# PaddlePaddle/MetaGym

Measured on NVIDIA H100. Metric: env-steps/sec (quadrotor 6-DoF, 65k envs), higher is better.
Workload: dtype f32

## Files before the change

### include/mgb200.h

```cpp
#ifndef MGB200_H
#define MGB200_H

#include <stdint.h>

#ifdef __cplusplus
extern "C" {
#endif

#define MGB_OK 0
#define MGB_ERR_ARG (-1)
#define MGB_ERR_CUDA (-2)
#define MGB_ERR_STATE (-3)


#define MGB_TASK_NO_COLLISION 0
#define MGB_TASK_HOVERING_CONTROL 1
#define MGB_TASK_VELOCITY_CONTROL 2

#define MGB_INTEGRATOR_REFERENCE 0
#define MGB_INTEGRATOR_RK4 1

#define MGB_FAIL_NONE 0
#define MGB_FAIL_RANGE 1
#define MGB_FAIL_VELOCITY 2
// ... 11 lines not shown
    double fail_velocity, fail_range, fail_w;
    float propeller[12];
    float propeller_norm[4];
    double min_voltage, max_voltage;
    float init_velocity[3];
    double init_velocity_noise;
    float init_angular_velocity[3];
    double init_angular_velocity_noise;
    double dt;
    int32_t nt;
    int32_t task;
    double healthy_reward;
    double z_offset;
    int32_t integrator;
    int32_t rk4_steps;
} mgb_quad_cfg;

typedef struct mgb_quad mgb_quad;

int mgb_quad_create(mgb_quad **out, int64_t n_envs, const mgb_quad_cfg *cfg, int device, int64_t env_index_base);
void mgb_quad_destroy(mgb_quad *h);

int mgb_quad_obs_dim(const mgb_quad *h);
int64_t mgb_quad_num_envs(const mgb_quad *h);

int mgb_quad_set_options(mgb_quad *h, int auto_reset, uint64_t seed);

int mgb_quad_set_map(mgb_quad *h, const int32_t *map_host, int32_t rows, int32_t cols);

int mgb_quad_set_targets(mgb_quad *h, const float *tbl_dev, int32_t n_tasks, const int32_t *env2task_dev);

int mgb_quad_make_targets(mgb_quad *h, const float *act_dev, int32_t n_tasks, float *tbl_dev, void *stream);

int mgb_quad_reset(mgb_quad *h, const uint8_t *mask_dev, const double *noise_dev, float *obs_dev, void *stream);

int mgb_quad_step(mgb_quad *h, const float *act_dev, float *obs_dev, float *rew_dev, uint8_t *done_dev,
                  int32_t *fail_dev, float *final_obs_dev, void *stream);
int mgb_quad_step_ex(mgb_quad *h, const float *act_dev, float *obs_dev, float *rew_dev, uint8_t *done_dev,
                     int32_t *fail_dev, float *final_obs_dev, uint8_t *truncated_dev, void *stream);

int mgb_quad_rollout(mgb_quad *h, int32_t T, const float *act_dev, uint64_t act_seed, float *act_out_dev,
                     float *obs_dev, float *rew_dev, uint8_t *done_dev, void *stream);
int mgb_quad_rollout_ex(mgb_quad *h, int32_t T, const float *act_dev, uint64_t act_seed, float *act_out_dev,
                        float *obs_dev, float *rew_dev, uint8_t *done_dev, float *final_obs_dev, uint8_t *truncated_dev,
                        void *stream);

#define MGB_ACT_TANH 0
#define MGB_ACT_RELU 1
#define MGB_POLICY_SAMPLE 0
#define MGB_POLICY_MEAN 1
#define MGB_POLICY_MAX_HIDDEN 3
#define MGB_POLICY_MAX_WIDTH 64

typedef struct mgb_policy {
    const float *params_dev;
    int32_t n_hidden;
    int32_t width[3];
    int32_t activation;
    int32_t mode;
} mgb_policy;

int mgb_quad_rollout_policy(mgb_quad *h, int32_t T, const mgb_policy *pol, uint64_t seed, float *act_out_dev,
                            float *logp_out_dev, float *obs0_out_dev, float *obs_dev, float *rew_dev, uint8_t *done_dev,
                            float *final_obs_dev, uint8_t *truncated_dev, void *stream);

int mgb_quad_step_host(mgb_quad *h, const float *act_host, float *obs_host, float *rew_host, uint8_t *done_host,
                       int32_t *fail_host, float *final_obs_host, void *stream);
int mgb_quad_step_host_ex(mgb_quad *h, const float *act_host, float *obs_host, float *rew_host, uint8_t *done_host,
                          int32_t *fail_host, float *final_obs_host, uint8_t *truncated_host, void *stream);

int mgb_quad_state(mgb_quad *h, float *state_dev, int32_t *ct_dev, int load, void *stream);

#define MGB_FINGERPRINT_WORDS 4
int64_t mgb_quad_record_bytes(const mgb_quad *h);
int mgb_quad_snapshot(mgb_quad *h, uint8_t *rec_dev, void *stream);
int mgb_quad_restore(mgb_quad *h, const uint8_t *rec_dev, int64_t n_rec, const int64_t *row_of_env_dev, void *stream);
int mgb_quad_counters(mgb_quad *h, uint64_t *t_base, int set);
int mgb_quad_fingerprint(const mgb_quad *h, uint64_t *out);

int64_t mgb_quad_launch_count(const mgb_quad *h);

const char *mgb_quad_step_kernel(const mgb_quad *h);


#define MGB_MAZE_2D 0
#define MGB_MAZE_DISCRETE_3D 1
#define MGB_MAZE_CONTINUOUS_3D 2

#define MGB_MAZE_SURVIVAL 0
#define MGB_MAZE_ESCAPE 1

#define MGB_OBS_U8 0
#define MGB_OBS_I32 1
#define MGB_OBS_F32 2

typedef struct mgb_maze_task_scalars {
    int32_t start[2];
    int32_t goal[2];
    double cell_size, wall_height, agent_height;
    double initial_life, max_life, step_reward, goal_reward;
} mgb_maze_task_scalars;

typedef struct mgb_maze_cfg {
    int32_t kind;
    int32_t task_type;
    int32_t n_cells;
    int32_t max_steps;
    int32_t view_grid;
    int32_t res_h;
    int32_t res_v;
    int32_t obs_dtype;
    double max_vision;
    double fov;
    double l_focal;
    double text_size;
} mgb_maze_cfg;

typedef struct mgb_maze mgb_maze;

int mgb_maze_create(mgb_maze **out, int64_t n_envs, const mgb_maze_cfg *cfg, int device, int64_t env_index_base);
void mgb_maze_destroy(mgb_maze *h);
int64_t mgb_maze_obs_bytes_per_env(const mgb_maze *h);

int mgb_maze_set_textures(mgb_maze *h, const uint8_t *grounds_host, int32_t n_tex, const uint8_t *ceil_host,
                          int32_t tex_size);

int mgb_maze_set_task(mgb_maze *h, int32_t n_tasks, const int8_t *walls_host, const int8_t *texts_host,
                      const double *food_rewards_host, const int32_t *food_interval_host,
                      const mgb_maze_task_scalars *scalars_host, const int32_t *env2task_host);

typedef struct mgb_maze_sampler_cfg {
    int32_t allow_loops, n_texts, food_interval, pad;
    double cell_size, wall_height, agent_height, step_reward;
    double goal_reward;
    double food_reward, initial_life, max_life, food_density, crowd_ratio;
} mgb_maze_sampler_cfg;

int mgb_maze_resample_tasks(mgb_maze *h, const uint8_t *mask_dev, const mgb_maze_sampler_cfg *cfg, uint64_t seed,
                            void *stream);

int mgb_maze_get_tasks(mgb_maze *h, int32_t count, const int32_t *task_slots_host, int8_t *walls_host, int8_t *texts_host,
                       double *food_rewards_host, int32_t *food_interval_host, mgb_maze_task_scalars *scalars_host);

int mgb_maze_set_cache(mgb_maze *h, int enabled);

int mgb_maze_cache_info(const mgb_maze *h, int64_t out[16]);

int mgb_maze_update_tasks(mgb_maze *h, int32_t count, const int32_t *task_slots_host, const int8_t *walls_host,
                          const int8_t *texts_host, const double *food_rewards_host, const int32_t *food_interval_host,
                          const mgb_maze_task_scalars *scalars_host, void *stream);

int mgb_maze_reset(mgb_maze *h, const uint8_t *mask_dev, void *obs_dev, void *stream);

int mgb_maze_step(mgb_maze *h, const void *act_dev, void *obs_dev, double *rew_dev, uint8_t *done_dev,
                  void *final_obs_dev, uint8_t *truncated_dev, void *stream);
int mgb_maze_set_options(mgb_maze *h, int auto_reset);

int mgb_maze_rollout(mgb_maze *h, int32_t T, const void *act_dev, uint64_t act_seed, void *act_out_dev,
                     void *obs_dev, double *rew_dev, uint8_t *done_dev, void *final_obs_dev, uint8_t *truncated_dev,
                     const mgb_maze_sampler_cfg *resample_cfg, uint64_t resample_seed, void *stream);

int mgb_maze_rollout_policy(mgb_maze *h, int32_t T, const mgb_policy *pol, uint64_t seed,
                            const mgb_maze_sampler_cfg *resample_cfg, uint64_t resample_seed, int32_t *act_out_dev,
                            float *logp_out_dev, float *obs0_out_dev, float *obs_dev, double *rew_dev, uint8_t *done_dev,
                            float *final_obs_dev, uint8_t *truncated_dev, void *stream);

// ... 67 lines not shown
```

### metagym_b200/_lib.py

```python
import ctypes
import os

PKG = os.path.dirname(os.path.abspath(__file__))
LIB_PATH = os.path.join(PKG, "libmgb200.so")

c_i32, c_i64, c_u64, c_f32, c_f64 = ctypes.c_int32, ctypes.c_int64, ctypes.c_uint64, ctypes.c_float, ctypes.c_double
vp = ctypes.c_void_p


class MgbError(RuntimeError):
    pass


class QuadCfg(ctypes.Structure):
    _fields_ = [
        ("precision", c_f64), ("quality", c_f64), ("inv_inertia", c_f32 * 9), ("drag_m", c_f32 * 3),
        ("drag_f", c_f32 * 3), ("gravity_center", c_f32 * 3), ("ct", c_f64 * 3), ("mm", c_f64), ("jm", c_f64),
        ("phi", c_f64), ("ra", c_f64), ("fail_velocity", c_f64), ("fail_range", c_f64), ("fail_w", c_f64),
        ("propeller", c_f32 * 12), ("propeller_norm", c_f32 * 4), ("min_voltage", c_f64), ("max_voltage", c_f64),
        ("init_velocity", c_f32 * 3), ("init_velocity_noise", c_f64), ("init_angular_velocity", c_f32 * 3),
        ("init_angular_velocity_noise", c_f64), ("dt", c_f64), ("nt", c_i32), ("task", c_i32),
        ("healthy_reward", c_f64), ("z_offset", c_f64), ("integrator", c_i32), ("rk4_steps", c_i32),
    ]


class MazeTaskScalars(ctypes.Structure):
    _fields_ = [("start", c_i32 * 2), ("goal", c_i32 * 2), ("cell_size", c_f64), ("wall_height", c_f64),
                ("agent_height", c_f64), ("initial_life", c_f64), ("max_life", c_f64), ("step_reward", c_f64),
                ("goal_reward", c_f64)]


class MazeSamplerCfg(ctypes.Structure):
    _fields_ = [("allow_loops", c_i32), ("n_texts", c_i32), ("food_interval", c_i32), ("pad", c_i32),
                ("cell_size", c_f64), ("wall_height", c_f64), ("agent_height", c_f64), ("step_reward", c_f64),
                ("goal_reward", c_f64), ("food_reward", c_f64), ("initial_life", c_f64), ("max_life", c_f64),
                ("food_density", c_f64), ("crowd_ratio", c_f64)]


class MazeCfg(ctypes.Structure):
    _fields_ = [("kind", c_i32), ("task_type", c_i32), ("n_cells", c_i32), ("max_steps", c_i32),
                ("view_grid", c_i32), ("res_h", c_i32), ("res_v", c_i32), ("obs_dtype", c_i32),
                ("max_vision", c_f64), ("fov", c_f64), ("l_focal", c_f64), ("text_size", c_f64)]


class Policy(ctypes.Structure):
    _fields_ = [("params_dev", vp), ("n_hidden", c_i32), ("width", c_i32 * 3), ("activation", c_i32), ("mode", c_i32)]


class RnnPolicy(ctypes.Structure):
    _fields_ = [("params_dev", vp), ("hidden", c_i32), ("feedback", c_i32), ("reset", c_i32), ("head_hidden", c_i32),
                ("head_width", c_i32), ("activation", c_i32), ("mode", c_i32), ("cell", c_i32)]


ACT_TANH, ACT_RELU = 0, 1
POLICY_SAMPLE, POLICY_MEAN = 0, 1
RNN_RESET_EPISODE, RNN_RESET_TASK = 0, 1
RNN_CELL_GRU, RNN_CELL_LSTM = 0, 1


SIGNATURES = {
    "mgb_quad_create": (ctypes.c_int, [ctypes.POINTER(vp), c_i64, ctypes.POINTER(QuadCfg), ctypes.c_int, c_i64]),
    "mgb_quad_destroy": (None, [vp]),
    "mgb_quad_obs_dim": (ctypes.c_int, [vp]),
    "mgb_quad_num_envs": (c_i64, [vp]),
    "mgb_quad_set_options": (ctypes.c_int, [vp, ctypes.c_int, c_u64]),
    "mgb_quad_set_map": (ctypes.c_int, [vp, vp, c_i32, c_i32]),
    "mgb_quad_set_targets": (ctypes.c_int, [vp, vp, c_i32, vp]),
    "mgb_quad_make_targets": (ctypes.c_int, [vp, vp, c_i32, vp, vp]),
    "mgb_quad_reset": (ctypes.c_int, [vp, vp, vp, vp, vp]),
    "mgb_quad_step": (ctypes.c_int, [vp, vp, vp, vp, vp, vp, vp, vp]),
    "mgb_quad_rollout": (ctypes.c_int, [vp, c_i32, vp, c_u64, vp, vp, vp, vp, vp]),
    "mgb_quad_step_host": (ctypes.c_int, [vp, vp, vp, vp, vp, vp, vp, vp]),
    "mgb_quad_step_ex": (ctypes.c_int, [vp, vp, vp, vp, vp, vp, vp, vp, vp]),
    "mgb_quad_step_host_ex": (ctypes.c_int, [vp, vp, vp, vp, vp, vp, vp, vp, vp]),
    "mgb_quad_rollout_ex": (ctypes.c_int, [vp, c_i32, vp, c_u64, vp, vp, vp, vp, vp, vp, vp]),
    "mgb_quad_rollout_policy": (ctypes.c_int, [vp, c_i32, ctypes.POINTER(Policy), c_u64, vp, vp, vp, vp, vp, vp, vp, vp,
                                               vp]),
    "mgb_quad_state": (ctypes.c_int, [vp, vp, vp, ctypes.c_int, vp]),
    "mgb_quad_launch_count": (c_i64, [vp]),
    "mgb_quad_step_kernel": (ctypes.c_char_p, [vp]),
    "mgb_maze_create": (ctypes.c_int, [ctypes.POINTER(vp), c_i64, ctypes.POINTER(MazeCfg), ctypes.c_int, c_i64]),
    "mgb_maze_destroy": (None, [vp]),
    "mgb_maze_obs_bytes_per_env": (c_i64, [vp]),
    "mgb_maze_set_textures": (ctypes.c_int, [vp, vp, c_i32, vp, c_i32]),
    "mgb_maze_set_task": (ctypes.c_int, [vp, c_i32, vp, vp, vp, vp, ctypes.POINTER(MazeTaskScalars), vp]),
    "mgb_maze_resample_tasks": (ctypes.c_int, [vp, vp, ctypes.POINTER(MazeSamplerCfg), c_u64, vp]),
    "mgb_maze_get_tasks": (ctypes.c_int, [vp, c_i32, vp, vp, vp, vp, vp, ctypes.POINTER(MazeTaskScalars)]),
    "mgb_maze_set_cache": (ctypes.c_int, [vp, ctypes.c_int]),
    "mgb_maze_cache_info": (ctypes.c_int, [vp, vp]),
    "mgb_maze_update_tasks": (ctypes.c_int, [vp, c_i32, vp, vp, vp, vp, vp, ctypes.POINTER(MazeTaskScalars), vp]),
    "mgb_maze_reset": (ctypes.c_int, [vp, vp, vp, vp]),
    "mgb_maze_step": (ctypes.c_int, [vp, vp, vp, vp, vp, vp, vp, vp]),
    "mgb_maze_set_options": (ctypes.c_int, [vp, ctypes.c_int]),
    "mgb_peer_alloc": (ctypes.c_int, [ctypes.c_int, c_u64, ctypes.POINTER(ctypes.c_void_p)]),
    "mgb_peer_free": (ctypes.c_int, [ctypes.c_int, vp]),
    "mgb_peer_export": (ctypes.c_int, [ctypes.c_int, vp, vp]),
    "mgb_peer_open": (ctypes.c_int, [ctypes.c_int, vp, ctypes.POINTER(ctypes.c_void_p)]),
    "mgb_peer_close": (ctypes.c_int, [ctypes.c_int, vp]),
    "mgb_quad_set_mirrors": (ctypes.c_int, [vp, ctypes.c_int, vp]),
    "mgb_maze_set_mirrors": (ctypes.c_int, [vp, ctypes.c_int, vp]),
    "mgb_quad_set_mirror_window": (ctypes.c_int, [vp, vp, c_u64]),
    "mgb_maze_set_mirror_window": (ctypes.c_int, [vp, vp, c_u64]),
    "mgb_quad_set_multicast": (ctypes.c_int, [vp, ctypes.c_int64]),
    "mgb_maze_set_multicast": (ctypes.c_int, [vp, ctypes.c_int64]),
    "mgb_maze_rollout": (ctypes.c_int, [vp, c_i32, vp, c_u64, vp, vp, vp, vp, vp, vp, ctypes.POINTER(MazeSamplerCfg),
                                        c_u64, vp]),
    "mgb_maze_rollout_policy": (ctypes.c_int, [vp, c_i32, ctypes.POINTER(Policy), c_u64, ctypes.POINTER(MazeSamplerCfg),
                                               c_u64, vp, vp, vp, vp, vp, vp, vp, vp, vp]),
    "mgb_maze_rollout_rnn": (ctypes.c_int, [vp, c_i32, ctypes.POINTER(RnnPolicy), c_u64, ctypes.POINTER(MazeSamplerCfg),
                                            c_u64, vp, vp, vp, vp, vp, vp, vp, vp, vp, vp, vp, vp]),
    "mgb_maze_pose": (ctypes.c_int, [vp, vp, vp, vp]),
    "mgb_maze_state": (ctypes.c_int, [vp, vp, vp, vp]),
    "mgb_maze_launch_count": (c_i64, [vp]),
    "mgb_maze_god_view": (ctypes.c_int, [vp, c_i32, vp, c_i32, c_i32, vp, vp]),
    "mgb_maze_set_path": (ctypes.c_int, [vp, ctypes.c_int]),
    "mgb_maze_path": (ctypes.c_int, [vp, c_i32, vp, vp, vp, vp]),
    "mgb_quad_record_bytes": (c_i64, [vp]),
    "mgb_quad_snapshot": (ctypes.c_int, [vp, vp, vp]),
    "mgb_quad_restore": (ctypes.c_int, [vp, vp, c_i64, vp, vp]),
    "mgb_quad_counters": (ctypes.c_int, [vp, ctypes.POINTER(c_u64), ctypes.c_int]),
    "mgb_quad_fingerprint": (ctypes.c_int, [vp, ctypes.POINTER(c_u64)]),
    "mgb_maze_record_bytes": (c_i64, [vp]),
    "mgb_maze_snapshot": (ctypes.c_int, [vp, vp, vp]),
    "mgb_maze_restore": (ctypes.c_int, [vp, vp, c_i64, vp, vp]),
    "mgb_maze_counters": (ctypes.c_int, [vp, ctypes.POINTER(c_u64), ctypes.c_int]),
    "mgb_maze_fingerprint": (ctypes.c_int, [vp, ctypes.POINTER(c_u64)]),
    "mgb_last_error": (ctypes.c_char_p, []),
    "mgb_version": (ctypes.c_char_p, []),
    "mgb_device_count": (ctypes.c_int, []),
}

_lib = None


def load():
    global _lib
    if _lib is not None:
        return _lib
    if not os.path.exists(LIB_PATH):
        raise MgbError("%s not found: build it with `python -m metagym_b200._build` (nvcc, sm_90a). "
                       "metagym_b200 has no CPU fallback." % LIB_PATH)
    lib = ctypes.CDLL(LIB_PATH)
    for name, (res, args) in SIGNATURES.items():
        fn = getattr(lib, name)
        fn.restype = res
        fn.argtypes = args
    _lib = lib
    return lib


def check(rc):
    if rc != 0:
        raise MgbError("libmgb200: %s (code %d)" % (load().mgb_last_error().decode(), rc))


def current_stream(torch, device):
    get = getattr(torch._C, "_cuda_getCurrentRawStream", None)
    if get is not None:
        return get(device.index)
    return torch.cuda.current_stream(device).cuda_stream


def ptr(t):
# ... 6 lines not shown
```

### metagym_b200/csrc/quad.cu

```cuda
#include <math.h>
#include <stdlib.h>
#include <string.h>
#include <memory>
#include <new>
#include <type_traits>
#include <utility>
#include <vector>

#include "mgb_common.cuh"
#include "mgb_policy.cuh"
#include "quad_lanes.cuh"

namespace {

constexpr int kThreads = 64;
constexpr int kMaxObs = 19;

struct QuadConst {
    float h;
    float k1phi;
    float k1;
    float inv_phi;
    float hjm;
    float hk;
    float mm;
    float ct0, ct1, ct2;
    float vmin, vmax;
    float A[4], B[4];
    float px[4], py[4], pz[4];
    float Df[3], Dm[3];
    float cg[3];
    float hI[9];
    float gm;
    float c_hm;
    float c_h2m;
    float fail_r2, fail_v2, fail_w2;
    float dt, healthy, z_off;
    float init_v[3], init_w[3], noise_v, noise_w;
    int nt, task, substeps, obs_dim;
    int rk4_steps;
    float rk4_h;
    float inv_jm, inv_m;
    float Iinv[9];
    int simple;
};

struct QuadArgs {
    float4 *planes;
    int64_t n_pad;
    int64_t n;
    int64_t env_base;
    const float *act;
    float *obs;
    float *rew;
    uint8_t *done;
    int32_t *fail;
    float *final_obs;
    const float4 *targets;
    int n_tasks;
    const int32_t *sat;
    int map_rows, map_cols, x_off, y_off;
    const int32_t *env2task;
    uint64_t seed;
    int auto_reset;
    int per_cta;
    int T;
    uint64_t act_seed;
    uint32_t t_base;
    float *act_out;
    MgbMirrors mir;
    uint8_t *truncated;
};

template <class T> struct VState {
    T p[3], v[3], om[3], w[4], R[9];
    int ct[Lanes<T>::N], ep[Lanes<T>::N];
};
using QState = VState<float>;

constexpr int kTileEnvs = 128;
constexpr int kPlanes = 6;

__device__ __forceinline__ float4 *tile_base(const QuadArgs &a, int64_t e)
{
    return a.planes + (e / kTileEnvs) * (kPlanes * kTileEnvs) + (e % kTileEnvs);
}

__device__ __forceinline__ void unpack_state(const float4 q[kPlanes], QState &s)
{
    s.p[0] = q[0].x; s.p[1] = q[0].y; s.p[2] = q[0].z; s.v[0] = q[0].w;
    s.v[1] = q[1].x; s.v[2] = q[1].y; s.om[0] = q[1].z; s.om[1] = q[1].w;
    s.om[2] = q[2].x; s.w[0] = q[2].y; s.w[1] = q[2].z; s.w[2] = q[2].w;
    s.w[3] = q[3].x; s.R[0] = q[3].y; s.R[1] = q[3].z; s.R[2] = q[3].w;
    s.R[3] = q[4].x; s.R[4] = q[4].y; s.R[5] = q[4].z; s.R[6] = q[4].w;
    s.R[7] = q[5].x; s.R[8] = q[5].y; s.ct[0] = __float_as_int(q[5].z); s.ep[0] = __float_as_int(q[5].w);
}
__device__ __forceinline__ void pack_state(const QState &s, float4 q[kPlanes])
{
    q[0] = make_float4(s.p[0], s.p[1], s.p[2], s.v[0]);
    q[1] = make_float4(s.v[1], s.v[2], s.om[0], s.om[1]);
    q[2] = make_float4(s.om[2], s.w[0], s.w[1], s.w[2]);
    q[3] = make_float4(s.w[3], s.R[0], s.R[1], s.R[2]);
    q[4] = make_float4(s.R[3], s.R[4], s.R[5], s.R[6]);
    q[5] = make_float4(s.R[7], s.R[8], __int_as_float(s.ct[0]), __int_as_float(s.ep[0]));
}

__device__ __forceinline__ void load_state(const QuadArgs &a, int64_t e, QState &s)
{
    const float4 *b = tile_base(a, e);
    float4 q[kPlanes];
#pragma unroll
    for (int k = 0; k < kPlanes; ++k) q[k] = b[k * kTileEnvs];
    unpack_state(q, s);
}

__device__ __forceinline__ void store_state(const QuadArgs &a, int64_t e, const QState &s)
{
    float4 *b = tile_base(a, e);
    float4 q[kPlanes];
    pack_state(s, q);
#pragma unroll
    for (int k = 0; k < kPlanes; ++k) b[k * kTileEnvs] = q[k];
}

template <class T> __device__ __forceinline__ void get_lane_state(const VState<T> &s, int h, QState &o);
template <class T> __device__ __forceinline__ void set_lane_state(VState<T> &s, int h, const QState &o);

__device__ __forceinline__ void load_state2(const QuadArgs &a, int64_t e, VState<f2> &s)
{
    QState s0, s1;
    load_state(a, e, s0);
    load_state(a, e + 1, s1);
    set_lane_state(s, 0, s0);
    set_lane_state(s, 1, s1);
}
__device__ __forceinline__ void store_state2(const QuadArgs &a, int64_t e, const VState<f2> &s)
{
    QState s0, s1;
    get_lane_state(s, 0, s0);
    get_lane_state(s, 1, s1);
    store_state(a, e, s0);
    store_state(a, e + 1, s1);
}

template <class T> __device__ __forceinline__ void get_lane_state(const VState<T> &s, int h, QState &o)
{
#pragma unroll
    for (int k = 0; k < 3; ++k) { o.p[k] = lane(s.p[k], h); o.v[k] = lane(s.v[k], h); o.om[k] = lane(s.om[k], h); }
#pragma unroll
    for (int k = 0; k < 4; ++k) o.w[k] = lane(s.w[k], h);
#pragma unroll
    for (int k = 0; k < 9; ++k) o.R[k] = lane(s.R[k], h);
    o.ct[0] = s.ct[h];
    o.ep[0] = s.ep[h];
// ... 607 lines not shown
                for (int k = 0; k < 9; ++k) set_lane(adj[k], h, adj1[k]);
                set_lane(id, h, id1);
                set_lane(power, h, pw1);
                fail[h] = f1[0];
            }
        }
    }
    if (!EARLY && vel) {
#pragma unroll
        for (int h = 0; h < N; ++h) prefetch_targets(c, a, task[h], ct_now[h], h, tr);
    }
    const bool state_first = N == 1 && STATE_FIRST && vel;
    if (state_first) {
        QState s1;
        get_lane_state(s, 0, s1);
        if (s1.ct[0] == c.nt || fail[0]) s1.ct[0] = 0;
        store_state(a, e, s1);
    }
    T o[kMaxObs], reward;
    int done[N], trunc[N];
    bool wf[N];
    finish_step(c, a, e, s, adj, id, z_old, x_old, y_old, power, fail, tr, o, reward, done, wf, trunc);
    bool stored = false;
    if constexpr (N == 2) {
        if (nact == 2) {
            store_state2(a, e, s);
            *reinterpret_cast<float2 *>(a.rew + e) = reward.v;
            *reinterpret_cast<uchar2 *>(a.done + e) = make_uchar2((uint8_t)done[0], (uint8_t)done[1]);
            if (a.fail) *reinterpret_cast<int2 *>(a.fail + e) = make_int2(fail[0], fail[1]);
            if (a.truncated) *reinterpret_cast<uchar2 *>(a.truncated + e) = make_uchar2((uint8_t)trunc[0], (uint8_t)trunc[1]);
            stored = true;
        }
    }
    if (!stored) {
#pragma unroll
        for (int h = 0; h < N; ++h) {
            if (h < nact) {
                QState s1;
                get_lane_state(s, h, s1);
                if (!state_first || wf[h]) store_state(a, e + h, s1);
                a.rew[e + h] = lane(reward, h);
                a.done[e + h] = (uint8_t)done[h];
                if (a.fail) a.fail[e + h] = fail[h];
                if (a.truncated) a.truncated[e + h] = (uint8_t)trunc[h];
            }
        }
    }
#pragma unroll
    for (int h = 0; h < N; ++h) {
        if (h < nact) {
            float *tr_h = trow + h * D;
            if (wf[h]) {
                if (a.final_obs) {
                    float *fr_h = frow + h * D;
#pragma unroll
                    for (int k = 0; k < 16; ++k) fr_h[k] = lane(o[k], h);
                    if (D == 19) { fr_h[16] = lane(o[16], h); fr_h[17] = lane(o[17], h); fr_h[18] = lane(o[18], h); }
                    final_mask |= 1 << h;
                }
                observe_reset(c, a, task[h], s, h, o);
            }
#pragma unroll
            for (int k = 0; k < 16; ++k) tr_h[k] = lane(o[k], h);
            if (D == 19) { tr_h[16] = lane(o[16], h); tr_h[17] = lane(o[17], h); tr_h[18] = lane(o[18], h); }
        }
    }
}

__device__ __forceinline__ void publish_final(const QuadArgs &a, const float *ftile, int64_t e, int local_row, int lanes,
                                              int final_mask, int D)
{
    if (!a.final_obs) return;
    if (__syncthreads_or(final_mask)) {
        for (int h = 0; h < lanes; ++h) {
            if (final_mask & (1 << h)) {
                float *dst = a.final_obs + (e + h) * D;
                const float *frow = ftile + (local_row + h) * D;
                for (int k = 0; k < D; ++k) dst[k] = frow[k];
            }
        }
    }
}

template <bool SIMPLE>
__global__ void __launch_bounds__(kThreads) quad_step_kernel(const __grid_constant__ QuadConst c,
                                                             const __grid_constant__ QuadArgs a)
{
    __shared__ __align__(128) float tile[kThreads * kMaxObs];
    __shared__ __align__(128) float ftile[kThreads * kMaxObs];
    const int64_t e0 = (int64_t)blockIdx.x * kThreads;
    const int64_t e = e0 + threadIdx.x;
    const int rows = (int)((a.n - e0) < kThreads ? (a.n - e0) : kThreads);
    const int D = c.obs_dim;
    const bool active = e < a.n;
    int final_mask = 0;

    asm volatile("griddepcontrol.launch_dependents;");
    const int task[1] = {active ? env_task(c, a, e) : 0};
    asm volatile("griddepcontrol.wait;" ::: "memory");

    if (active) {
        QState s;
        load_state(a, e, s);
        const float4 act = __ldg(reinterpret_cast<const float4 *>(a.act) + e);
        const float V[4] = {act.x, act.y, act.z, act.w};
        step_body<SIMPLE, false, true, float>(c, a, e, 1, s, V, task, tile + threadIdx.x * D, ftile + threadIdx.x * D,
                                              final_mask);
    }
    publish_tile(a.obs, tile, e0, rows, D);
    publish_final(a, ftile, e, threadIdx.x, 1, final_mask, D);
    if (threadIdx.x == 0) mgb_bulk_wait_read<0>();
}

template <bool SIMPLE>
__global__ void __launch_bounds__(512, 1) quad_step_wide_kernel(const __grid_constant__ QuadConst c,
                                                                const __grid_constant__ QuadArgs a)
{
    extern __shared__ __align__(128) float wide_smem[];
    const int per = a.per_cta;
    float *tile = wide_smem, *ftile = wide_smem + (size_t)per * kMaxObs;
    const int64_t e0 = (int64_t)blockIdx.x * per;
    const int64_t e = e0 + threadIdx.x;
    int rows = (int)((a.n - e0) < per ? (a.n - e0) : per);
    if (rows < 0) rows = 0;
    const int D = c.obs_dim;
    const bool active = (int)threadIdx.x < rows;
    int final_mask = 0;
    asm volatile("griddepcontrol.launch_dependents;");
    const int task[1] = {active ? env_task(c, a, e) : 0};
    asm volatile("griddepcontrol.wait;" ::: "memory");
    if (active) {
        QState s;
        load_state(a, e, s);
        const float4 act = __ldg(reinterpret_cast<const float4 *>(a.act) + e);
        const float V[4] = {act.x, act.y, act.z, act.w};
        step_body<SIMPLE, false, false, float>(c, a, e, 1, s, V, task, tile + threadIdx.x * D, ftile + threadIdx.x * D,
                                               final_mask);
    }
    if (rows > 0) publish_tile(a.obs, tile, e0, rows, D);
    else __syncthreads();
    publish_final(a, ftile, e, threadIdx.x, 1, final_mask, D);
    if (threadIdx.x == 0) mgb_bulk_wait_read<0>();
}

template <bool SIMPLE>
__global__ void __launch_bounds__(256, 1) quad_step2_kernel(const __grid_constant__ QuadConst c,
                                                            const __grid_constant__ QuadArgs a)
{
    extern __shared__ __align__(128) float pair_smem[];
    const int per = a.per_cta;
    float *tile = pair_smem, *ftile = pair_smem + (size_t)per * kMaxObs;
    const int64_t e0 = (int64_t)blockIdx.x * per;
    int rows = (int)((a.n - e0) < per ? (a.n - e0) : per);
    if (rows < 0) rows = 0;
    const int le = 2 * (int)threadIdx.x;
    const int64_t e = e0 + le;
    const int D = c.obs_dim;
    const int nact = rows - le >= 2 ? 2 : (rows - le > 0 ? 1 : 0);
    int final_mask = 0;
    asm volatile("griddepcontrol.launch_dependents;");
    asm volatile("griddepcontrol.wait;" ::: "memory");
    if (nact > 0) {
        VState<f2> s;
        load_state2(a, e, s);
        const float4 a0 = __ldg(reinterpret_cast<const float4 *>(a.act) + e);
        const float4 a1 = nact == 2 ? __ldg(reinterpret_cast<const float4 *>(a.act) + e + 1) : make_float4(0.f, 0.f, 0.f, 0.f);
        const f2 V[4] = {pack2(a0.x, a1.x), pack2(a0.y, a1.y), pack2(a0.z, a1.z), pack2(a0.w, a1.w)};
        const int task[2] = {env_task(c, a, e), env_task(c, a, nact == 2 ? e + 1 : e)};
        step_body<SIMPLE, true, false, f2>(c, a, e, nact, s, V, task, tile + le * D, ftile + le * D, final_mask);
    }
    if (rows > 0) publish_tile(a.obs, tile, e0, rows, D);
    else __syncthreads();
// ... 251 lines not shown
    load_state(a, e, s);
    float *row = state + e * 22;
    if (load) {
        for (int k = 0; k < 3; ++k) { s.p[k] = row[k]; s.v[k] = row[3 + k]; s.om[k] = row[6 + k]; }
        for (int k = 0; k < 4; ++k) s.w[k] = row[9 + k];
        for (int k = 0; k < 9; ++k) s.R[k] = row[13 + k];
        if (ct) s.ct[0] = ct[e];
        store_state(a, e, s);
    } else {
        for (int k = 0; k < 3; ++k) { row[k] = s.p[k]; row[3 + k] = s.v[k]; row[6 + k] = s.om[k]; }
        for (int k = 0; k < 4; ++k) row[9 + k] = s.w[k];
        for (int k = 0; k < 9; ++k) row[13 + k] = s.R[k];
        if (ct) ct[e] = s.ct[0];
    }
}

__global__ void quad_init_kernel(QuadArgs a)
{
    const int64_t e = (int64_t)blockIdx.x * blockDim.x + threadIdx.x;
    if (e >= a.n_pad) return;
    QState s;
    for (int k = 0; k < 3; ++k) s.p[k] = s.v[k] = s.om[k] = 0.f;
    for (int k = 0; k < 4; ++k) s.w[k] = 0.f;
    for (int k = 0; k < 9; ++k) s.R[k] = (k % 4 == 0) ? 1.f : 0.f;
    s.ct[0] = 0;
    s.ep[0] = 0;
    store_state(a, e, s);
}

template <bool SIMPLE>
__global__ void quad_targets_kernel(const __grid_constant__ QuadConst c, const float *__restrict__ act, int n_tasks,
                                    float *__restrict__ tbl)
{
    const int k = blockIdx.x * blockDim.x + threadIdx.x;
    if (k >= n_tasks) return;
    QState s;
    for (int q = 0; q < 3; ++q) s.p[q] = s.v[q] = s.om[q] = 0.f;
    for (int q = 0; q < 4; ++q) s.w[q] = 0.f;
    for (int q = 0; q < 9; ++q) s.R[q] = (q % 4 == 0) ? 1.f : 0.f;
    s.ct[0] = 0; s.ep[0] = 0;
    float adj[9], id, power;
    adjugate(s.R, adj, id);
    for (int t = 0; t < c.nt; ++t) {
        const float4 a4 = reinterpret_cast<const float4 *>(act)[(int64_t)k * c.nt + t];
        const int fail = integrate1<SIMPLE>(c, s, a4, adj, id, power);
        float *dst = tbl + ((int64_t)k * c.nt + t) * 3;
        dst[0] = s.v[0]; dst[1] = s.v[1]; dst[2] = s.v[2];
        if (fail) {
            for (int r = t + 1; r < c.nt; ++r) {
                float *d2 = tbl + ((int64_t)k * c.nt + r) * 3;
                d2[0] = d2[1] = d2[2] = __int_as_float(0x7fc00000);
            }
            return;
        }
    }
}

__global__ void quad_targets_layout_kernel(const float *__restrict__ src, int nt, int n_tasks, float4 *__restrict__ dst)
{
    const int64_t i = (int64_t)blockIdx.x * blockDim.x + threadIdx.x;
    if (i >= (int64_t)nt * n_tasks) return;
    const int64_t t = i / n_tasks, k = i % n_tasks;
    const float *s = src + (k * nt + t) * 3;
    dst[i] = make_float4(s[0], s[1], s[2], 0.f);
}

}

struct QuadStaging {
    MgbDev<float> d_act, d_obs, d_rew, d_final;
    MgbDev<uint8_t> d_done, d_trunc;
    MgbDev<int32_t> d_fail;
    MgbPinned<float> h_act, h_obs, h_rew, h_final;
    MgbPinned<uint8_t> h_done, h_trunc;
    MgbPinned<int32_t> h_fail;
};

struct mgb_quad {
    int device = 0;
    int64_t n = 0, n_pad = 0, env_base = 0;
    mgb_quad_cfg cfg;
    QuadConst c;
    MgbDev<float4> planes;
    MgbDev<int32_t> sat;
    int map_rows = 0, map_cols = 0, x_off = 0, y_off = 0;
    MgbDev<float4> targets;
    MgbDev<int32_t> env2task;
    int n_tasks = 0;
    int auto_reset = 0;
    int num_sms = 132;
    int wide_kernel = -1;
    int packed = 0;
    int stream_kernel = 1;
    int pdl = 1;
    int zerocopy = 1;
    uint64_t seed = 0;
    uint32_t t_base = 0;
    int64_t launches = 0;
    uint64_t fp_map = 0, fp_targets = 0;
    MgbMirrors mir = {};
    MgbMirrorWindow mir_win;
    QuadStaging stage;
};

static QuadArgs base_args(const mgb_quad *h)
{
    QuadArgs a;
    memset(&a, 0, sizeof(a));
    a.planes = h->planes.get();
    a.n_pad = h->n_pad;
    a.n = h->n;
    a.env_base = h->env_base;
    a.targets = h->targets.get();
    a.n_tasks = h->n_tasks;
    a.sat = h->sat.get(); a.map_rows = h->map_rows; a.map_cols = h->map_cols; a.x_off = h->x_off; a.y_off = h->y_off;
    a.env2task = h->env2task.get();
    a.seed = h->seed;
    a.auto_reset = h->auto_reset;
    return a;
}

template <class F> static auto with_simple(const mgb_quad *h, F &&f)
{
    return h->c.simple ? f(std::true_type()) : f(std::false_type());
}

static int derive_constants(const mgb_quad_cfg *g, QuadConst *c)
{
    memset(c, 0, sizeof(*c));
    c->h = (float)g->precision;
    c->k1 = (float)(g->phi / g->ra);
    c->k1phi = (float)(g->phi / g->ra * g->phi);
    c->inv_phi = (float)(1.0 / g->phi);
    c->hjm = (float)(g->precision / g->jm);
    c->hk = (float)(g->precision / g->jm * (g->phi / g->ra * g->phi));
    c->mm = (float)g->mm;
    c->ct0 = (float)g->ct[0]; c->ct1 = (float)g->ct[1]; c->ct2 = (float)g->ct[2];
    c->vmin = (float)g->min_voltage; c->vmax = (float)g->max_voltage;
    bool simple = (g->ct[2] == 0.0);
    for (int i = 0; i < 4; ++i) {
        c->px[i] = g->propeller[3 * i]; c->py[i] = g->propeller[3 * i + 1]; c->pz[i] = g->propeller[3 * i + 2];
        c->A[i] = (float)((double)c->py[i] * (double)g->propeller_norm[i]);
        c->B[i] = (float)((double)c->px[i] * (double)g->propeller_norm[i]);
        if (c->pz[i] != 0.f) simple = false;
    }
    for (int k = 0; k < 3; ++k) {
        c->Df[k] = g->drag_f[k]; c->Dm[k] = g->drag_m[k]; c->cg[k] = g->gravity_center[k];
        if (c->cg[k] != 0.f) simple = false;
        c->init_v[k] = g->init_velocity[k]; c->init_w[k] = g->init_angular_velocity[k];
    }
    for (int k = 0; k < 9; ++k) {
        c->hI[k] = (float)(g->precision * (double)g->inv_inertia[k]);
        if (k % 4 != 0 && g->inv_inertia[k] != 0.f) simple = false;
    }
    c->gm = (float)((double)(float)-9.8 * g->quality);
    c->c_hm = (float)(g->precision / g->quality);
    c->c_h2m = (float)(0.5 * g->precision * g->precision / g->quality);
    c->fail_r2 = (float)(g->fail_range * g->fail_range);
    c->fail_v2 = (float)(g->fail_velocity * g->fail_velocity);
    c->fail_w2 = (float)(g->fail_w * g->fail_w);
    c->dt = (float)g->dt; c->healthy = (float)g->healthy_reward; c->z_off = (float)g->z_offset;
    c->noise_v = (float)g->init_velocity_noise; c->noise_w = (float)g->init_angular_velocity_noise;
    c->nt = g->nt; c->task = g->task;
    c->substeps = (int)(g->dt / g->precision);
    c->rk4_steps = g->integrator == MGB_INTEGRATOR_RK4 ? (g->rk4_steps > 0 ? g->rk4_steps : 1) : 0;
    c->rk4_h = c->rk4_steps ? (float)(g->dt / c->rk4_steps) : 0.f;
    c->inv_jm = (float)(1.0 / g->jm);
    c->inv_m = (float)(1.0 / g->quality);
    for (int k = 0; k < 9; ++k) c->Iinv[k] = g->inv_inertia[k];
    c->obs_dim = g->task == MGB_TASK_VELOCITY_CONTROL ? 19 : 16;
    c->simple = simple ? 1 : 0;
    return 0;
}

extern "C" int mgb_quad_create(mgb_quad **out, int64_t n_envs, const mgb_quad_cfg *cfg, int device,
                               int64_t env_index_base)
{
    MGB_REQUIRE(out && cfg, "null argument");
    MGB_REQUIRE(n_envs > 0, "n_envs must be positive");
    MGB_REQUIRE(cfg->task >= 0 && cfg->task <= 2, "invalid task");
    MGB_REQUIRE(cfg->nt > 0, "nt must be positive");
    MGB_REQUIRE(!(cfg->precision < 1e-8 || cfg->precision > cfg->dt), "Inproper parameter of precision");
    int ndev = 0;
    MGB_CUDA(cudaGetDeviceCount(&ndev));
    MGB_REQUIRE(device >= 0 && device < ndev, "device index out of range");
    MgbDeviceGuard guard(device);
    std::unique_ptr<mgb_quad> h(new (std::nothrow) mgb_quad());
    MGB_REQUIRE(h, "out of host memory");
    h->device = device;
    h->n = n_envs;
    h->n_pad = (n_envs + 127) / 128 * 128;
    h->env_base = env_index_base;
    h->cfg = *cfg;
    derive_constants(cfg, &h->c);
    if (const char *ev = getenv("MGB_PDL")) h->pdl = atoi(ev) != 0;
    {
        cudaDeviceProp prop;
        if (cudaGetDeviceProperties(&prop, device) == cudaSuccess) h->num_sms = prop.multiProcessorCount;
    }
    if (const char *ev = getenv("MGB_HOST_ZEROCOPY")) h->zerocopy = atoi(ev);
    if (const char *ev = getenv("MGB_STREAM_KERNEL")) h->stream_kernel = atoi(ev) != 0;
    if (const char *ev = getenv("MGB_PACKED")) h->packed = atoi(ev) != 0;
    if (const char *ev = getenv("MGB_WIDE_KERNEL")) h->wide_kernel = atoi(ev) != 0;
    {
        const int max_smem = 512 * kMaxObs * 4 * 2;
        with_simple(h.get(), [&](auto simple) {
            cudaFuncSetAttribute(quad_step_wide_kernel<simple>, cudaFuncAttributeMaxDynamicSharedMemorySize, max_smem);
            cudaFuncSetAttribute(quad_step2_kernel<simple>, cudaFuncAttributeMaxDynamicSharedMemorySize, max_smem);
        });
        if (cudaGetLastError() != cudaSuccess) {
            mgb_set_error("cudaFuncSetAttribute(quad_step_wide_kernel, %d bytes of shared memory) failed", max_smem);
            return MGB_ERR_CUDA;
        }
    }
    MGB_CUDA(h->planes.alloc(sizeof(float4) * 6 * h->n_pad));
    quad_init_kernel<<<(unsigned)((h->n_pad + 255) / 256), 256>>>(base_args(h.get()));
    MGB_CUDA(cudaDeviceSynchronize());
    h->launches += 1;
    *out = h.release();
    return MGB_OK;
}

extern "C" void mgb_quad_destroy(mgb_quad *h)
{
    if (!h) return;
    MgbDeviceGuard guard(h->device);
    cudaDeviceSynchronize();
    delete h;
}

extern "C" int mgb_quad_obs_dim(const mgb_quad *h) { return h ? h->c.obs_dim : MGB_ERR_ARG; }
extern "C" int64_t mgb_quad_num_envs(const mgb_quad *h) { return h ? h->n : MGB_ERR_ARG; }
extern "C" int64_t mgb_quad_launch_count(const mgb_quad *h) { return h ? h->launches : MGB_ERR_ARG; }

extern "C" int mgb_quad_set_options(mgb_quad *h, int auto_reset, uint64_t seed)
{
    MGB_REQUIRE(h, "null handle");
    h->auto_reset = auto_reset ? 1 : 0;
    h->seed = seed;
    return MGB_OK;
}

extern "C" int mgb_quad_set_map(mgb_quad *h, const int32_t *map_host, int32_t rows, int32_t cols)
{
    MGB_REQUIRE(h, "null handle");
    MgbDeviceGuard guard(h->device);
    MGB_CUDA(cudaDeviceSynchronize());
    if (!map_host) {
        h->sat.reset();
        h->map_rows = h->map_cols = h->x_off = h->y_off = 0;
        h->fp_map = 0;
        return MGB_OK;
    }
    MGB_REQUIRE(h->c.task != MGB_TASK_VELOCITY_CONTROL, "velocity_control has no map (env.py:101-104)");
    MGB_REQUIRE(rows > 0 && cols > 0 && rows <= 8192 && cols <= 8192, "map size out of range");
    int starts = 0, sr = 0, sc = 0;
    for (int r = 0; r < rows; ++r)
        for (int q = 0; q < cols; ++q)
            if (map_host[(size_t)r * cols + q] == -1) { ++starts; sr = r; sc = q; }
    MGB_REQUIRE(starts == 1, "the map must mark exactly one start cell with -1 (env.py:108-109)");
    std::vector<int32_t> sat((size_t)(rows + 1) * (cols + 1), 0);
    for (int r = 0; r < rows; ++r)
        for (int q = 0; q < cols; ++q) {
            const int v = (r == sr && q == sc) ? 0 : map_host[(size_t)r * cols + q];
            sat[(size_t)(r + 1) * (cols + 1) + q + 1] = (v != 0 ? 1 : 0) + sat[(size_t)r * (cols + 1) + q + 1] +
                                                        sat[(size_t)(r + 1) * (cols + 1) + q] - sat[(size_t)r * (cols + 1) + q];
        }
    MgbDev<int32_t> d_sat;
    MGB_CUDA(d_sat.alloc(sat.size() * sizeof(int32_t)));
    MGB_CUDA(cudaMemcpy(d_sat.get(), sat.data(), sat.size() * sizeof(int32_t), cudaMemcpyHostToDevice));
    h->sat = std::move(d_sat);
    h->map_rows = rows; h->map_cols = cols; h->x_off = sc; h->y_off = sr;
    h->fp_map = mgb_fnv(mgb_fnv(mgb_fnv(MGB_FNV_BASIS, &rows, sizeof(rows)), &cols, sizeof(cols)), map_host,
                        (size_t)rows * cols * sizeof(int32_t));
    return MGB_OK;
}

extern "C" int mgb_quad_set_targets(mgb_quad *h, const float *tbl_dev, int32_t n_tasks, const int32_t *env2task_dev)
{
    MGB_REQUIRE(h && tbl_dev && env2task_dev, "null argument");
    MGB_REQUIRE(n_tasks > 0, "n_tasks must be positive");
    MgbDeviceGuard guard(h->device);
    MGB_CUDA(cudaDeviceSynchronize());
    const int64_t rows = (int64_t)h->c.nt * n_tasks;
    MgbDev<float4> targets;
    MgbDev<int32_t> env2task;
    MGB_CUDA(targets.alloc(sizeof(float4) * (size_t)rows));
    MGB_CUDA(env2task.alloc(sizeof(int32_t) * h->n));
    quad_targets_layout_kernel<<<(unsigned)((rows + 255) / 256), 256>>>(tbl_dev, h->c.nt, n_tasks, targets.get());
    MGB_CUDA(cudaGetLastError());
    MGB_CUDA(cudaMemcpy(env2task.get(), env2task_dev, sizeof(int32_t) * h->n, cudaMemcpyDeviceToDevice));
    MGB_CUDA(cudaDeviceSynchronize());
    std::vector<float4> tbl((size_t)rows);
    MGB_CUDA(cudaMemcpy(tbl.data(), targets.get(), tbl.size() * sizeof(float4), cudaMemcpyDeviceToHost));
    h->targets = std::move(targets); h->env2task = std::move(env2task);
    h->n_tasks = n_tasks;
    h->fp_targets = mgb_fnv(mgb_fnv(MGB_FNV_BASIS, &n_tasks, sizeof(n_tasks)), tbl.data(), tbl.size() * sizeof(float4));
    return MGB_OK;
}

static int check_ready(const mgb_quad *h)
{
    if (h->c.task == MGB_TASK_VELOCITY_CONTROL && !h->targets) {
        mgb_set_error("velocity_control: call mgb_quad_set_targets before reset/step");
        return MGB_ERR_STATE;
    }
    return MGB_OK;
}

extern "C" int mgb_quad_make_targets(mgb_quad *h, const float *act_dev, int32_t n_tasks, float *tbl_dev, void *stream)
{
    MgbRange nvtx_range("mgb_quad_make_targets");
    MGB_REQUIRE(h && act_dev && tbl_dev, "null argument");
    MGB_REQUIRE(n_tasks > 0, "n_tasks must be positive");
    MgbDeviceGuard guard(h->device);
    cudaStream_t st = (cudaStream_t)stream;
    const int threads = 32, blocks = (n_tasks + threads - 1) / threads;
    with_simple(h, [&](auto simple) {
        quad_targets_kernel<simple><<<blocks, threads, 0, st>>>(h->c, act_dev, n_tasks, tbl_dev);
    });
    MGB_CUDA(cudaGetLastError());
    h->launches += 1;
    return MGB_OK;
}

extern "C" int mgb_quad_reset(mgb_quad *h, const uint8_t *mask_dev, const double *noise_dev, float *obs_dev,
                              void *stream)
{
    MgbRange nvtx_range("mgb_quad_reset");
    MGB_REQUIRE(h, "null handle");
    int rc = check_ready(h);
    if (rc) return rc;
    MgbDeviceGuard guard(h->device);
    QuadArgs a = base_args(h);
    a.obs = obs_dev;
    quad_reset_kernel<<<(unsigned)((h->n + kThreads - 1) / kThreads), kThreads, 0, (cudaStream_t)stream>>>(
        h->c, a, mask_dev, noise_dev);
    MGB_CUDA(cudaGetLastError());
    h->launches += 1;
    return MGB_OK;
}

struct StepPlan {
    void (*kernel)(QuadConst, QuadArgs);
    const char *name;
    dim3 grid, block;
    size_t smem = 0;
    int per_cta = 0;
};

static StepPlan plan_step(const mgb_quad *h, const QuadArgs &a)
{
#define STEP_KERNEL(k) k<simple>, simple ? #k "<true>" : #k "<false>"
    return with_simple(h, [&](auto simple) {
        const unsigned blocks = (unsigned)((a.n + kThreads - 1) / kThreads);
        const bool act16 = (reinterpret_cast<uintptr_t>(a.act) & 15u) == 0;
        if (h->stream_kernel && (int64_t)blocks > (int64_t)h->num_sms * 32 && act16)
            return StepPlan{STEP_KERNEL(quad_stream_kernel), dim3((unsigned)(h->num_sms * 4)), dim3(kStreamThreads)};
        const bool packed = h->packed && h->c.rk4_steps == 0 && a.n >= 2 && act16 &&
                            (reinterpret_cast<uintptr_t>(a.rew) & 7u) == 0 && (reinterpret_cast<uintptr_t>(a.done) & 1u) == 0 &&
                            (reinterpret_cast<uintptr_t>(a.fail) & 7u) == 0 && (reinterpret_cast<uintptr_t>(a.truncated) & 1u) == 0;
        const bool single_wave = a.n <= (int64_t)h->num_sms * 512 && a.n >= (int64_t)h->num_sms * 64;
        const int64_t wide_max = (int64_t)h->num_sms * (h->wide_kernel > 0 ? 512 : 384);
        if (!packed && !(h->wide_kernel != 0 && single_wave && a.n <= wide_max))
            return StepPlan{STEP_KERNEL(quad_step_kernel), dim3(blocks), dim3(kThreads)};
        int per = single_wave ? (int)((a.n + h->num_sms - 1) / h->num_sms) : a.n < (int64_t)h->num_sms * 64 ? 64 : 256;
        per = (per + 3) / 4 * 4;
        const dim3 grid((unsigned)((a.n + per - 1) / per)), block((unsigned)((per / (packed ? 2 : 1) + 31) / 32 * 32));
        const size_t smem = (size_t)per * kMaxObs * 4 * 2;
        if (packed) return StepPlan{STEP_KERNEL(quad_step2_kernel), grid, block, smem, per};
        return StepPlan{STEP_KERNEL(quad_step_wide_kernel), grid, block, smem, per};
    });
#undef STEP_KERNEL
}

static int launch_step(mgb_quad *h, QuadArgs a, cudaStream_t st)
{
    const StepPlan p = plan_step(h, a);
    a.per_cta = p.per_cta;
    cudaLaunchConfig_t cfg;
    memset(&cfg, 0, sizeof(cfg));
    cfg.gridDim = p.grid;
    cfg.blockDim = p.block;
    cfg.dynamicSmemBytes = p.smem;
    cfg.stream = st;
    cudaLaunchAttribute attr[1];
    attr[0].id = cudaLaunchAttributeProgrammaticStreamSerialization;
    attr[0].val.programmaticStreamSerializationAllowed = h->pdl ? 1 : 0;
    cfg.attrs = attr;
    cfg.numAttrs = 1;
    MGB_CUDA(cudaLaunchKernelEx(&cfg, p.kernel, h->c, a));
    MGB_CUDA(cudaGetLastError());
    h->launches += 1;
    return MGB_OK;
}

extern "C" const char *mgb_quad_step_kernel(const mgb_quad *h) { return h ? plan_step(h, base_args(h)).name : ""; }

static int step_dev(mgb_quad *h, const float *act_dev, float *obs_dev, float *rew_dev, uint8_t *done_dev,
                    int32_t *fail_dev, float *final_obs_dev, uint8_t *truncated_dev, void *stream)
{
    MGB_REQUIRE(h && act_dev && obs_dev && rew_dev && done_dev, "null argument");
    MGB_REQUIRE((reinterpret_cast<uintptr_t>(act_dev) & 15u) == 0, "act_dev must be 16-byte aligned");
    int rc = check_ready(h);
    if (rc) return rc;
    MgbDeviceGuard guard(h->device);
    QuadArgs a = base_args(h);
    a.act = act_dev; a.obs = obs_dev; a.rew = rew_dev; a.done = done_dev; a.fail = fail_dev;
    a.final_obs = final_obs_dev;
    a.truncated = truncated_dev;
    return launch_step(h, a, (cudaStream_t)stream);
}

extern "C" int mgb_quad_step(mgb_quad *h, const float *act_dev, float *obs_dev, float *rew_dev, uint8_t *done_dev,
                             int32_t *fail_dev, float *final_obs_dev, void *stream)
{
    MgbRange nvtx_range("mgb_quad_step");
    return step_dev(h, act_dev, obs_dev, rew_dev, done_dev, fail_dev, final_obs_dev, nullptr, stream);
}

extern "C" int mgb_quad_step_ex(mgb_quad *h, const float *act_dev, float *obs_dev, float *rew_dev, uint8_t *done_dev,
                                int32_t *fail_dev, float *final_obs_dev, uint8_t *truncated_dev, void *stream)
{
    MgbRange nvtx_range("mgb_quad_step_ex");
    return step_dev(h, act_dev, obs_dev, rew_dev, done_dev, fail_dev, final_obs_dev, truncated_dev, stream);
}

static int rollout(mgb_quad *h, int32_t T, const float *act_dev, uint64_t act_seed, float *act_out_dev, float *obs_dev,
                   float *rew_dev, uint8_t *done_dev, float *final_obs_dev, uint8_t *truncated_dev, void *stream)
{
    MGB_REQUIRE(h, "null handle");
    MGB_REQUIRE(T > 0, "T must be positive");
    MGB_REQUIRE((reinterpret_cast<uintptr_t>(act_dev) & 15u) == 0, "act_dev must be 16-byte aligned");
    const bool fin = final_obs_dev || truncated_dev;
    MGB_REQUIRE(!final_obs_dev || h->auto_reset, "final_obs needs auto_reset on (without it obs already is the terminal observation)");
    MGB_REQUIRE(!fin || h->mir.count == 0,
                "final_obs / truncated are not delivered through output mirrors or multicast (set_mirrors([]) first)");
    int rc = check_ready(h);
    if (rc) return rc;
    MgbDeviceGuard guard(h->device);
    QuadArgs a = base_args(h);
    a.act = act_dev; a.obs = obs_dev; a.rew = rew_dev; a.done = done_dev;
    a.T = T; a.act_seed = act_seed; a.t_base = h->t_base; a.act_out = act_out_dev;
    a.final_obs = final_obs_dev; a.truncated = truncated_dev;
    const unsigned blocks = (unsigned)((a.n + kThreads - 1) / kThreads);
    a.mir = h->mir;
    if (h->mir.count != 0)
        MGB_REQUIRE(h->mir_win.holds_rollout((uint64_t)T * h->n, obs_dev, (uint64_t)h->c.obs_dim * 4, rew_dev, 4, done_dev,
                                             act_out_dev, 16),
                    "mirrors are on but an output lies outside the mirrored arena (set_mirrors([]) first)");
    const int xm = h->mir.count == MGB_MIRROR_MULTICAST ? 2 : h->mir.count > 0 ? 1 : 0;
    if (xm == 2) {
        MGB_REQUIRE(h->n % 4 == 0, "multicast outputs need num_envs % 4 == 0");
        MGB_REQUIRE((((uintptr_t)done_dev | (uintptr_t)rew_dev | (uintptr_t)obs_dev) & 3) == 0 && ((uintptr_t)act_out_dev & 15) == 0,
                    "multicast outputs must be 4-byte (actions: 16-byte) aligned");
    }
    const auto kernel = with_simple(h, [&](auto simple) {
        return xm == 2 ? quad_rollout_kernel<simple, 2, false> : xm == 1 ? quad_rollout_kernel<simple, 1, false>
               : fin   ? quad_rollout_kernel<simple, 0, true>  : quad_rollout_kernel<simple, 0, false>;
    });
    kernel<<<blocks, kThreads, 0, (cudaStream_t)stream>>>(h->c, a, MgbMlp{});
    MGB_CUDA(cudaGetLastError());
    h->t_base += (uint32_t)T;
    h->launches += 1;
    return MGB_OK;
}

extern "C" int mgb_quad_rollout_policy(mgb_quad *h, int32_t T, const mgb_policy *pol, uint64_t seed, float *act_out_dev,
                                       float *logp_out_dev, float *obs0_out_dev, float *obs_dev, float *rew_dev,
                                       uint8_t *done_dev, float *final_obs_dev, uint8_t *truncated_dev, void *stream)
{
    MgbRange nvtx_range("mgb_quad_rollout_policy");
    MGB_REQUIRE(h, "null handle");
    MGB_REQUIRE(T > 0, "T must be positive");
    MgbMlp m;
// ... 317 lines not shown
```

Baseline: 8.733 billion.

## Chain consecutive step launches per tile with release/acquire flags instead of grid-wide PDL wait

```diff
diff --git a/include/mgb200.h b/include/mgb200.h
--- a/include/mgb200.h
+++ b/include/mgb200.h
@@ -117,6 +117,8 @@
 
 const char *mgb_quad_step_kernel(const mgb_quad *h);
 
+int64_t mgb_quad_chain_fallbacks(const mgb_quad *h);
+
 
 #define MGB_MAZE_2D 0
 #define MGB_MAZE_DISCRETE_3D 1
diff --git a/metagym_b200/_lib.py b/metagym_b200/_lib.py
--- a/metagym_b200/_lib.py
+++ b/metagym_b200/_lib.py
@@ -79,6 +79,7 @@
     "mgb_quad_state": (ctypes.c_int, [vp, vp, vp, ctypes.c_int, vp]),
     "mgb_quad_launch_count": (c_i64, [vp]),
     "mgb_quad_step_kernel": (ctypes.c_char_p, [vp]),
+    "mgb_quad_chain_fallbacks": (c_i64, [vp]),
     "mgb_maze_create": (ctypes.c_int, [ctypes.POINTER(vp), c_i64, ctypes.POINTER(MazeCfg), ctypes.c_int, c_i64]),
     "mgb_maze_destroy": (None, [vp]),
     "mgb_maze_obs_bytes_per_env": (c_i64, [vp]),
diff --git a/metagym_b200/csrc/quad.cu b/metagym_b200/csrc/quad.cu
--- a/metagym_b200/csrc/quad.cu
+++ b/metagym_b200/csrc/quad.cu
@@ -70,6 +70,8 @@
     float *act_out;
     MgbMirrors mir;
     uint8_t *truncated;
+    uint32_t *chain;
+    int obs_reused;
 };
 
 template <class T> struct VState {
@@ -843,12 +845,98 @@
     }
 }
 
+__device__ __forceinline__ uint32_t ld_acquire(const uint32_t *p)
+{
+    uint32_t v;
+    asm volatile("ld.acquire.gpu.global.u32 %0, [%1];" : "=r"(v) : "l"(p) : "memory");
+    return v;
+}
+__device__ __forceinline__ void st_release(uint32_t *p, uint32_t v)
+{
+    asm volatile("st.release.gpu.global.u32 [%0], %1;" ::"l"(p), "r"(v) : "memory");
+}
+constexpr int kChainPolls = 1 << 18;
+__device__ __forceinline__ bool chain_poll(const uint32_t *w, uint32_t want)
+{
+    for (int i = 0; i < kChainPolls; ++i) {
+        if (ld_acquire(w) == want) return true;
+        __nanosleep(64);
+    }
+    return false;
+}
+
 template <bool SIMPLE>
-__global__ void __launch_bounds__(kThreads) quad_step_kernel(const __grid_constant__ QuadConst c,
-                                                             const __grid_constant__ QuadArgs a)
+__device__ __forceinline__ void step_chained(const QuadConst &c, const QuadArgs &a, float *tile, float *ftile)
+{
+    static_assert(kTileEnvs == 2 * kThreads, "a CTA steps the two halves of one state tile");
+    __shared__ int s_wait;
+    __shared__ uint32_t s_ticket;
+    uint32_t *w = a.chain + 3 * (int64_t)blockIdx.x;
+    const int64_t t0 = (int64_t)blockIdx.x * kTileEnvs;
+    const int D = c.obs_dim;
+    const int tid = threadIdx.x;
+    if (tid == 0) {
+        const uint32_t ticket = atomicAdd(w, 1u);
+        s_ticket = ticket;
+        s_wait = ld_acquire(w + 2) == ticket;
+    }
+    asm volatile("griddepcontrol.launch_dependents;" ::: "memory");
+    const int task0 = t0 + tid < a.n ? env_task(c, a, t0 + tid) : 0;
+    const int task1 = t0 + kThreads + tid < a.n ? env_task(c, a, t0 + kThreads + tid) : 0;
+    __syncthreads();
+    bool waited = s_wait != 0;
+    if (waited) asm volatile("griddepcontrol.wait;" ::: "memory");
+#pragma unroll 1
+    for (int h = 0; h < 2; ++h) {
+        if (!waited) {
+            if (tid == 0 && !chain_poll(w + 1 + h, s_ticket)) {
+                asm volatile("griddepcontrol.wait;" ::: "memory");
+                atomicAdd(a.chain + 3 * (int64_t)gridDim.x, 1u);
+                s_wait = 1;
+            }
+            __syncthreads();
+            if (s_wait) {
+                waited = true;
+                asm volatile("griddepcontrol.wait;" ::: "memory");
+            }
+        }
+        const int64_t e0 = t0 + h * kThreads, e = e0 + tid;
+        const int64_t left = a.n - e0;
+        const int rows = left <= 0 ? 0 : left < kThreads ? (int)left : kThreads;
+        int final_mask = 0;
+        if (tid < rows) {
+            QState s;
+            load_state(a, e, s);
+            const float4 act = __ldg(reinterpret_cast<const float4 *>(a.act) + e);
+            const float V[4] = {act.x, act.y, act.z, act.w};
+            const int task[1] = {h == 0 ? task0 : task1};
+            step_body<SIMPLE, false, true, float>(c, a, e, 1, s, V, task, tile + tid * D, ftile + tid * D, final_mask);
+        }
+        if (rows > 0) publish_tile(a.obs, tile, e0, rows, D);
+        publish_final(a, ftile, e, tid, 1, final_mask, D);
+        if (tid == 0) {
+            if (h == 1 || a.obs_reused) {
+                mgb_bulk_wait<0>();
+                asm volatile("fence.proxy.async.global;" ::: "memory");
+            } else {
+                mgb_bulk_wait_read<0>();
+            }
+        }
+        __syncthreads();
+        if (tid == 0) st_release(w + 1 + h, s_ticket + 1u);
+    }
+}
+
+template <bool SIMPLE, bool CHAIN = false>
+__global__ void __launch_bounds__(kThreads, CHAIN ? 8 : 1) quad_step_kernel(const __grid_constant__ QuadConst c,
+                                                                            const __grid_constant__ QuadArgs a)
 {
     __shared__ __align__(128) float tile[kThreads * kMaxObs];
     __shared__ __align__(128) float ftile[kThreads * kMaxObs];
+    if constexpr (CHAIN) {
+        step_chained<SIMPLE>(c, a, tile, ftile);
+        return;
+    }
     const int64_t e0 = (int64_t)blockIdx.x * kThreads;
     const int64_t e = e0 + threadIdx.x;
     const int rows = (int)((a.n - e0) < kThreads ? (a.n - e0) : kThreads);
@@ -1266,6 +1354,8 @@
     mgb_quad_cfg cfg;
     QuadConst c;
     MgbDev<float4> planes;
+    MgbDev<uint32_t> chain;
+    const float *chain_obs = nullptr;
     MgbDev<int32_t> sat;
     int map_rows = 0, map_cols = 0, x_off = 0, y_off = 0;
     MgbDev<float4> targets;
@@ -1286,6 +1376,8 @@
     MgbMirrorWindow mir_win;
     QuadStaging stage;
 };
+
+static size_t chain_bytes(int64_t n_pad) { return sizeof(uint32_t) * (size_t)(3 * (n_pad / kTileEnvs) + 1); }
 
 static QuadArgs base_args(const mgb_quad *h)
 {
@@ -1398,6 +1490,8 @@
         }
     }
     MGB_CUDA(h->planes.alloc(sizeof(float4) * 6 * h->n_pad));
+    MGB_CUDA(h->chain.alloc(chain_bytes(h->n_pad)));
+    MGB_CUDA(cudaMemset(h->chain.get(), 0, chain_bytes(h->n_pad)));
     quad_init_kernel<<<(unsigned)((h->n_pad + 255) / 256), 256>>>(base_args(h.get()));
     MGB_CUDA(cudaDeviceSynchronize());
     h->launches += 1;
@@ -1411,6 +1505,15 @@
     MgbDeviceGuard guard(h->device);
     cudaDeviceSynchronize();
     delete h;
+}
+
+extern "C" int64_t mgb_quad_chain_fallbacks(const mgb_quad *h)
+{
+    MGB_REQUIRE(h, "null handle");
+    MgbDeviceGuard guard(h->device);
+    uint32_t v = 0;
+    MGB_CUDA(cudaMemcpy(&v, h->chain.get() + 3 * (h->n_pad / kTileEnvs), sizeof(v), cudaMemcpyDeviceToHost));
+    return (int64_t)v;
 }
 
 extern "C" int mgb_quad_obs_dim(const mgb_quad *h) { return h ? h->c.obs_dim : MGB_ERR_ARG; }
@@ -1531,6 +1634,7 @@
     dim3 grid, block;
     size_t smem = 0;
     int per_cta = 0;
+    bool chained = false;
 };
 
 static StepPlan plan_step(const mgb_quad *h, const QuadArgs &a)
@@ -1546,8 +1650,15 @@
                             (reinterpret_cast<uintptr_t>(a.fail) & 7u) == 0 && (reinterpret_cast<uintptr_t>(a.truncated) & 1u) == 0;
         const bool single_wave = a.n <= (int64_t)h->num_sms * 512 && a.n >= (int64_t)h->num_sms * 64;
         const int64_t wide_max = (int64_t)h->num_sms * (h->wide_kernel > 0 ? 512 : 384);
-        if (!packed && !(h->wide_kernel != 0 && single_wave && a.n <= wide_max))
+        if (!packed && !(h->wide_kernel != 0 && single_wave && a.n <= wide_max)) {
+            const int64_t tiles = h->n_pad / kTileEnvs;
+            if constexpr (decltype(simple)::value) {
+                if (tiles <= (int64_t)h->num_sms * 4 && a.n > (int64_t)h->num_sms * 384)
+                    return StepPlan{quad_step_kernel<true, true>, "quad_step_kernel<true>", dim3((unsigned)tiles),
+                                    dim3(kThreads), 0, 0, true};
+            }
             return StepPlan{STEP_KERNEL(quad_step_kernel), dim3(blocks), dim3(kThreads)};
+        }
         int per = single_wave ? (int)((a.n + h->num_sms - 1) / h->num_sms) : a.n < (int64_t)h->num_sms * 64 ? 64 : 256;
         per = (per + 3) / 4 * 4;
         const dim3 grid((unsigned)((a.n + per - 1) / per)), block((unsigned)((per / (packed ? 2 : 1) + 31) / 32 * 32));
@@ -1562,6 +1673,8 @@
 {
     const StepPlan p = plan_step(h, a);
     a.per_cta = p.per_cta;
+    a.chain = p.chained ? h->chain.get() : nullptr;
+    a.obs_reused = p.chained && a.obs == h->chain_obs;
     cudaLaunchConfig_t cfg;
     memset(&cfg, 0, sizeof(cfg));
     cfg.gridDim = p.grid;
@@ -1575,6 +1688,7 @@
     cfg.numAttrs = 1;
     MGB_CUDA(cudaLaunchKernelEx(&cfg, p.kernel, h->c, a));
     MGB_CUDA(cudaGetLastError());
+    h->chain_obs = p.chained ? a.obs : nullptr;
     h->launches += 1;
     return MGB_OK;
 }
```

Result: faster. 9.320 billion, median of 6 (+6.7%).
